# AidaDSP/aidadsp-lv2

Hardware: AMD Instinct MI355X
Metric: audio samples/sec (48 kHz mono, many streams) (higher is better)
Workload: dtype f32; 1 GPU; cfg2: LSTM-32 amp model, 1024 streams/GPU x 256-frame blocks, full run() chain, TTL-default controls; streams_per_gpu=1024, frames=256, kernel=k_lstm_pipe4<32>

## Files before the change

aidadsp-lv2_amd/csrc/aidax_device.h:

```cpp
#pragma once

#include <hip/hip_runtime.h>

#include <cfloat>

#include "aidax_layout.h"

namespace aidax {

__device__ __forceinline__ float dpp_row_shr1(float v)
{
    return __builtin_bit_cast(float, __builtin_amdgcn_update_dpp(0, __builtin_bit_cast(int, v), 0x111, 0xf, 0xf, true));
}

template <int CTRL, int ROW_MASK>
__device__ __forceinline__ float dpp_take(float v)
{
    return __builtin_bit_cast(float, __builtin_amdgcn_update_dpp(0, __builtin_bit_cast(int, v), CTRL, ROW_MASK, 0xf, ROW_MASK == 0xf));
}

__device__ __forceinline__ float wave_sum(float v)
{
    v = v + dpp_take<0xB1, 0xf>(v);
    v = v + dpp_take<0x4E, 0xf>(v);
    v = v + dpp_take<0x141, 0xf>(v);
    v = v + dpp_take<0x140, 0xf>(v);
    v = v + dpp_take<0x142, 0xa>(v);
    v = v + dpp_take<0x143, 0xc>(v);
    return __builtin_bit_cast(float, __builtin_amdgcn_readlane(__builtin_bit_cast(int, v), 63));
}

template <int N>
__device__ __forceinline__ void fmac_row_ror(float& acc, float h, float w)
{
    static_assert(N >= 1 && N <= 15, "rotation within a row of 16 lanes");
    asm volatile("v_fmac_f32_dpp %0, %1, %2 row_ror:%3 row_mask:0xf bank_mask:0xf" : "+v"(acc) : "v"(h), "v"(w), "n"(N));
}

#define AIDAX_ROR1(N, W) "v_fmac_f32_dpp %0, %1, %" #W " row_ror:" #N " row_mask:0xf bank_mask:0xf\n\t"
__device__ __forceinline__ void fmac_row_ror_1_15(float& a0, float h, const float* w)
{
    asm volatile(AIDAX_ROR1(1, 2) AIDAX_ROR1(2, 3) AIDAX_ROR1(3, 4) AIDAX_ROR1(4, 5) AIDAX_ROR1(5, 6) AIDAX_ROR1(6, 7) AIDAX_ROR1(7, 8)
                 AIDAX_ROR1(8, 9) AIDAX_ROR1(9, 10) AIDAX_ROR1(10, 11) AIDAX_ROR1(11, 12) AIDAX_ROR1(12, 13) AIDAX_ROR1(13, 14)
                 AIDAX_ROR1(14, 15) AIDAX_ROR1(15, 16)
                 : "+v"(a0)
                 : "v"(h), "v"(w[1]), "v"(w[2]), "v"(w[3]), "v"(w[4]), "v"(w[5]), "v"(w[6]), "v"(w[7]), "v"(w[8]), "v"(w[9]),
                   "v"(w[10]), "v"(w[11]), "v"(w[12]), "v"(w[13]), "v"(w[14]), "v"(w[15]));
}
#undef AIDAX_ROR1

typedef float aidax_f32x2 __attribute__((ext_vector_type(2)));
#define AIDAX_PKA(ACC, W, HQ) "v_pk_fma_f32 %" #ACC ", %" #W ", %" #HQ ", %" #ACC " op_sel_hi:[1,0,1]\n\t"
#define AIDAX_PKB(ACC, W, HQ) "v_pk_fma_f32 %" #ACC ", %" #W ", %" #HQ ", %" #ACC " op_sel:[0,1,0] op_sel_hi:[1,1,1]\n\t"
#define AIDAX_PKA0(ACC, W, HQ) "v_pk_fma_f32 %" #ACC ", %" #W ", %" #HQ ", 0 op_sel_hi:[1,0,0]\n\t"
#define AIDAX_PKB0(ACC, W, HQ) "v_pk_fma_f32 %" #ACC ", %" #W ", %" #HQ ", 0 op_sel:[0,1,0] op_sel_hi:[1,1,0]\n\t"
__device__ __forceinline__ aidax_f32x2 pk_fma_lds16(aidax_f32x2 pA, const aidax_f32x2* w, const aidax_f32x2* hq)
{
    aidax_f32x2 pB, pC, pD;
    asm volatile(AIDAX_PKA(0, 4, 20) AIDAX_PKB0(1, 5, 20) AIDAX_PKA0(2, 6, 21) AIDAX_PKB0(3, 7, 21)
                 AIDAX_PKA(0, 8, 22) AIDAX_PKB(1, 9, 22) AIDAX_PKA(2, 10, 23) AIDAX_PKB(3, 11, 23)
                 AIDAX_PKA(0, 12, 24) AIDAX_PKB(1, 13, 24) AIDAX_PKA(2, 14, 25) AIDAX_PKB(3, 15, 25)
                 AIDAX_PKA(0, 16, 26) AIDAX_PKB(1, 17, 26) AIDAX_PKA(2, 18, 27) AIDAX_PKB(3, 19, 27)
                 "v_pk_add_f32 %0, %0, %1\n\t"
                 "v_pk_add_f32 %2, %2, %3"
                 : "+v"(pA), "=&v"(pB), "=&v"(pC), "=&v"(pD)
                 : "v"(w[0]), "v"(w[1]), "v"(w[2]), "v"(w[3]), "v"(w[4]), "v"(w[5]), "v"(w[6]), "v"(w[7]), "v"(w[8]), "v"(w[9]), "v"(w[10]),
                   "v"(w[11]), "v"(w[12]), "v"(w[13]), "v"(w[14]), "v"(w[15]),
                   "v"(hq[0]), "v"(hq[1]), "v"(hq[2]), "v"(hq[3]), "v"(hq[4]), "v"(hq[5]), "v"(hq[6]), "v"(hq[7]));
    return pA + pC;
}
#undef AIDAX_PKA
#undef AIDAX_PKB
#undef AIDAX_PKA0
#undef AIDAX_PKB0

struct Pair { float lo, hi; };

__device__ __forceinline__ Pair share_halves(float v)
{
    const unsigned u = __builtin_bit_cast(unsigned, v);
    const auto r = __builtin_amdgcn_permlane32_swap(u, u, false, false);
    const unsigned r0 = r[0], r1 = r[1];
    return { __builtin_bit_cast(float, r0), __builtin_bit_cast(float, r1) };
}

__device__ __forceinline__ Pair share_rows(float v)
{
    const unsigned u = __builtin_bit_cast(unsigned, v);
    const auto r = __builtin_amdgcn_permlane16_swap(u, u, false, false);
    const unsigned r0 = r[0], r1 = r[1];
    return { __builtin_bit_cast(float, r0), __builtin_bit_cast(float, r1) };
}

__device__ __forceinline__ float fast_sigmoid(float v)
{
    const float e = __builtin_amdgcn_exp2f(v * -1.44269504088896340736f);
    return __builtin_amdgcn_rcpf(1.0f + e);
}

constexpr float kNegLog2e = -1.44269504088896340736f;
__device__ __forceinline__ float sigmoid_pre(float v_scaled)
{
    return __builtin_amdgcn_rcpf(1.0f + __builtin_amdgcn_exp2f(v_scaled));
}


constexpr float kTanhP[7] = { 0.9999999933888696f, 0.13084010352004496f, 0.003103956503888039f, 1.1154311501654368e-05f,
                              -2.0225239996482085e-08f, 5.277955823366522e-11f, -8.488730763828322e-14f };
constexpr float kTanhQ[4] = { 1.0f, 0.46417337453820245f, 0.02449517952619233f, 0.00025461456545097517f };
constexpr float kTanhClamp = 0x1.f9b3c2p+2f;
__device__ __forceinline__ float tanh_rat_clamp(float v) { return __builtin_fminf(__builtin_fmaxf(v, -kTanhClamp), kTanhClamp); }
template <bool kUFirst = false>
__device__ __forceinline__ float tanh_rat(float v)
{
    const float x = tanh_rat_clamp(v);
    const float u = x * x;
#ifndef AIDAX_TANH_PLAIN
    typedef float f32x2_t __attribute__((ext_vector_type(2)));
    const f32x2_t uu = { u, u };
    auto step = [&](f32x2_t pq, f32x2_t c) { return kUFirst ? __builtin_elementwise_fma(uu, pq, c) : __builtin_elementwise_fma(pq, uu, c); };
    f32x2_t pq = { kTanhP[6], kTanhQ[3] };
    pq = step(pq, f32x2_t{ kTanhP[5], kTanhQ[2] });
    pq = step(pq, f32x2_t{ kTanhP[4], kTanhQ[1] });
    pq = step(pq, f32x2_t{ kTanhP[3], kTanhQ[0] });
    float pp = pq.x;
    pp = __builtin_fmaf(pp, u, kTanhP[2]);
    pp = __builtin_fmaf(pp, u, kTanhP[1]);
    pp = __builtin_fmaf(pp, u, kTanhP[0]);
    return (pp * x) * __builtin_amdgcn_rcpf(pq.y);
#endif
    float p = kTanhP[6];
    p = __builtin_fmaf(p, u, kTanhP[5]);
    p = __builtin_fmaf(p, u, kTanhP[4]);
    p = __builtin_fmaf(p, u, kTanhP[3]);
    p = __builtin_fmaf(p, u, kTanhP[2]);
    p = __builtin_fmaf(p, u, kTanhP[1]);
    p = __builtin_fmaf(p, u, kTanhP[0]);
    float q = kTanhQ[3];
    q = __builtin_fmaf(q, u, kTanhQ[2]);
    q = __builtin_fmaf(q, u, kTanhQ[1]);
    q = __builtin_fmaf(q, u, kTanhQ[0]);
    return (p * x) * __builtin_amdgcn_rcpf(q);
}

__device__ __forceinline__ float tanh_exp(float v)
{
    const float e = __builtin_amdgcn_exp2f(v * 2.88539008177792681472f);
    return __builtin_fmaf(-2.0f, __builtin_amdgcn_rcpf(1.0f + e), 1.0f);
}

__device__ __forceinline__ float tanh_exp_pre(float v_scaled)
{
    return __builtin_fmaf(-2.0f, __builtin_amdgcn_rcpf(1.0f + __builtin_amdgcn_exp2f(v_scaled)), 1.0f);
}

struct ExpRamp {
    float mem, coef, tc;
    __device__ __forceinline__ void arm(float m, float target, float c)
    {
        mem = m; coef = c; tc = target * (1.f - c);
    }
    __device__ __forceinline__ float next() { mem = mem * coef + tc; return mem; }
};

__device__ __forceinline__ float lin_next(float& mem, float target, float step)
{
    const float y0 = mem;
    const float dy = target - y0;
    mem = y0 + __builtin_copysignf(__builtin_fminf(__builtin_fabsf(dy), __builtin_fabsf(step)), dy);
    return mem;
}

__device__ __forceinline__ bool eq_stage_transparent(double a0, double a1, double a2, double b1, double b2, double z1, double z2)
{
    return a0 == 1.0 && a1 == b1 && a2 == b2 && z1 == 0.0 && z2 == 0.0;
}
__device__ __forceinline__ float eq_skip_sample(float y, float& p)
{
    const float o = y + p;
    p = p + (y - y);
    return o;
}

struct ChainPass {
    int K, gain_lane;
    bool active;
    double a0, a1, a2, b1, b2, z1, z2;
    ExpRamp g;
    bool eq_skip;
    float eq_p;
};

template <int DST_STRIDE, bool CHECK>
__device__ __forceinline__ void chain_step(ChainPass& c, int stage, bool run, bool writer, float head, float& carry,
                                           float* dst, int s, int n)
{
    const float from_left = dpp_row_shr1(carry);
    const float x = stage == 0 ? head : from_left;
// ... 453 lines not shown
```

aidadsp-lv2_amd/csrc/aidax_kernels.hip:

```cpp
#include <hip/hip_runtime.h>
#include <hip/hip_ext.h>

#include <cfloat>

#include <mutex>
#include "aidax_device.h"
#include "aidax_kernels.h"
#include "aidax_layout.h"

namespace aidax {

template <int H, bool ROTP = true>
struct LstmCell {
    static constexpr LaneMap M = lstm_map(H);
    static constexpr int S = M.S, SLOTS = M.slots, NU = M.NU, GPL = M.GPL;
    static constexpr int PACK = lstm_pack_regs(H);
    static constexpr int STATE = 2 * H;
    static constexpr bool ROT4 = ROTP && lstm_rot4(H);
    static constexpr int KW = lstm_row_weights(H, ROT4);

    float w[NU][GPL][KW];
    typedef float f32x2 __attribute__((ext_vector_type(2)));
    f32x2 wl2[16];
    float wx[NU][GPL][kMaxInputs];
    float bias[NU][GPL];
    float wd[NU], bd;
    float aka[GPL], akb[GPL];
    float c[NU], h[NU];
    int part, slot;
#ifdef AIDAX_PIPE_TRACE
    unsigned long long ts6 = 0;
    unsigned long long ts[6];
#define PT_STAMP(k) do { if constexpr (TR) { __builtin_amdgcn_sched_barrier(0); ts[k] = __builtin_amdgcn_s_memtime(); __builtin_amdgcn_sched_barrier(0); } } while (0)
#else
#define PT_STAMP(k) do { } while (0)
#endif
    static constexpr int kStatePart = S == 2 ? 1 : 0;
    static constexpr bool ROT = ROTP && lstm_rot2(H);
    static constexpr int kPackOffset = (!ROTP && lstm_has_alt_pack(H)) ? lstm_alt_pack_offset(H) : 0;

    __device__ __forceinline__ void load(const float* __restrict__ wbase, const float* __restrict__ st, int lane)
    {
        const float* __restrict__ wp = wbase + kPackOffset;
        part = lane / SLOTS;
        slot = lane % SLOTS;
        int r = 0;
#pragma unroll
        for (int m = 0; m < NU; ++m)
#pragma unroll
            for (int e = 0; e < GPL; ++e) {
#pragma unroll
                for (int k = 0; k < KW; ++k) w[m][e][k] = wp[(r++) * kWave + lane];
#pragma unroll
                for (int i = 0; i < kMaxInputs; ++i) wx[m][e][i] = wp[(r++) * kWave + lane];
                bias[m][e] = wp[(r++) * kWave + lane];
            }
#pragma unroll
        for (int m = 0; m < NU; ++m) wd[m] = wp[(r++) * kWave + lane];
        bd = wp[(r++) * kWave + lane];
        if constexpr (ROTP && lstm_rot2(H)) {
            constexpr int kRow = KW + kMaxInputs + 1;
#pragma unroll
            for (int k = 0; k < 16; ++k) wl2[k] = f32x2{ wp[(16 + k) * kWave + lane], wp[(kRow + 16 + k) * kWave + lane] };
        }
#pragma unroll
        for (int e = 0; e < GPL; ++e) {
            const bool is_tanh = (part + S * e) == 2;
            aka[e] = is_tanh ? 1.f : 0.5f;
            akb[e] = is_tanh ? 0.f : 0.5f;
        }
#pragma unroll
        for (int m = 0; m < NU; ++m) {
            const int j = slot + m * SLOTS;
            h[m] = j < H ? st[j] : 0.f;
            c[m] = j < H ? st[H + j] : 0.f;
        }
    }

    __device__ __forceinline__ void store(float* __restrict__ st) const
    {
#pragma unroll
        for (int m = 0; m < NU; ++m) {
            const int j = slot + m * SLOTS;
            if (part == kStatePart && j < H) { st[j] = h[m]; st[H + j] = c[m]; }
        }
    }

    __device__ __forceinline__ void publish_h(float* hbuf) const
    {
#pragma unroll
        for (int m = 0; m < NU; ++m) {
            const int j = slot + m * SLOTS;
            if constexpr (S == 2 && !ROT) {
                if (j < H) hbuf[part == kStatePart ? j : H] = h[m];
            } else {
                if (j < H) hbuf[j] = h[m];
            }
        }
    }

    static constexpr int HID = H;

    __device__ __forceinline__ float dense_partial() const
    {
        float d = 0.f;
#pragma unroll
        for (int m = 0; m < NU; ++m) d = __builtin_fmaf(wd[m], h[m], d);
        return d;
    }

    template <int NI = kMaxInputs, int WINDOW = 0, bool TR = false>
    __device__ __forceinline__ void step(float x0, float x1, float x2, const float* hprev, float* hout)
    {
        PT_STAMP(0);
        float acc[NU][GPL];
#pragma unroll
        for (int m = 0; m < NU; ++m)
#pragma unroll
            for (int e = 0; e < GPL; ++e) {
                float a = bias[m][e];
                a = __builtin_fmaf(wx[m][e][0], x0, a);
                if constexpr (NI >= 2) a = __builtin_fmaf(wx[m][e][1], x1, a);
                if constexpr (NI >= 3) a = __builtin_fmaf(wx[m][e][2], x2, a);
                acc[m][e] = a;
            }
        if constexpr (ROT4) {
            const float hr = h[0];
            float a0 = __builtin_fmaf(w[0][0][0], hr, acc[0][0]);
            fmac_row_ror_1_15(a0, hr, w[0][0]);
            acc[0][0] = a0;
            (void)hprev;
        } else if constexpr (ROT) {
            const float4* hv = reinterpret_cast<const float4*>(hprev + 16 * (1 - ((slot >> 4) & 1)));
            const float4 q0 = hv[0], q1 = hv[1], q2 = hv[2], q3 = hv[3];
            __builtin_amdgcn_sched_barrier(0);
            const float hr = h[0];
            float a0 = acc[0][0], a1 = acc[0][1];
            a0 = __builtin_fmaf(w[0][0][0], hr, a0);
            a1 = __builtin_fmaf(w[0][1][0], hr, a1);
            fmac_row_ror_1_15(a0, hr, w[0][0]);
            fmac_row_ror_1_15(a1, hr, w[0][1]);
            __builtin_amdgcn_s_waitcnt(0xc07f);
            PT_STAMP(1);
            const f32x2 hq[8] = { f32x2{ q0.x, q0.y }, f32x2{ q0.z, q0.w }, f32x2{ q1.x, q1.y }, f32x2{ q1.z, q1.w },
                                  f32x2{ q2.x, q2.y }, f32x2{ q2.z, q2.w }, f32x2{ q3.x, q3.y }, f32x2{ q3.z, q3.w } };
            const f32x2 a01 = pk_fma_lds16(f32x2{ a0, a1 }, wl2, hq);
            acc[0][0] = a01.x; acc[0][1] = a01.y;
            PT_STAMP(2);
        } else {
        const float4* hv = reinterpret_cast<const float4*>(hprev);
#pragma unroll
        for (int k4 = 0; k4 < H / 4; ++k4) {
            const float4 q = hv[k4];
#pragma unroll
            for (int m = 0; m < NU; ++m)
#pragma unroll
                for (int e = 0; e < GPL; ++e) {
                    float a = acc[m][e];
                    a = __builtin_fmaf(w[m][e][4 * k4 + 0], q.x, a);
                    a = __builtin_fmaf(w[m][e][4 * k4 + 1], q.y, a);
                    a = __builtin_fmaf(w[m][e][4 * k4 + 2], q.z, a);
                    a = __builtin_fmaf(w[m][e][4 * k4 + 3], q.w, a);
                    acc[m][e] = a;
                }
            if constexpr (WINDOW > 0) { if ((k4 + 1) % WINDOW == 0) __builtin_amdgcn_sched_barrier(0); }
        }
        }
        __builtin_amdgcn_wave_barrier();
#pragma unroll
        for (int m = 0; m < NU; ++m) {
            float act[GPL];
#pragma unroll
            for (int e = 0; e < GPL; ++e) {
                if constexpr (S == 1) {
                    act[e] = e == 2 ? tanh_rat<ROT>(acc[m][e]) : sigmoid_pre(acc[m][e]);
                } else if (S == 2 && e == 0) {
                    act[e] = sigmoid_pre(acc[m][e]);
                } else {
                    act[e] = __builtin_fmaf(tanh_rat<ROT>(acc[m][e]), aka[e], akb[e]);
                }
            }
            PT_STAMP(3);
            float gi_gg, gf, go;
            if constexpr (S == 1) {
                gi_gg = act[0] * act[2]; gf = act[1]; go = act[3];
            } else if constexpr (S == 2) {
                const float ig = act[0] * act[1];
                const auto r = __builtin_amdgcn_permlane32_swap(__builtin_bit_cast(unsigned, acc[m][1]), __builtin_bit_cast(unsigned, ig), false, false);
                const unsigned r0 = r[0];
                gi_gg = __builtin_bit_cast(float, r0); gf = act[0]; go = act[1];
            } else {
                const Pair p = share_halves(act[0]);
                const Pair lo = share_rows(p.lo), hi = share_rows(p.hi);
                gi_gg = lo.lo * hi.lo; gf = lo.hi; go = hi.hi;
            }
            const float cn = __builtin_fmaf(gf, c[m], gi_gg);
            c[m] = cn;
#ifdef AIDAX_TANHC_EXP
            const float hn = go * tanh_exp(cn);
#else
            const float hn = go * tanh_rat<ROT>(cn);
#endif
            if constexpr (ROT) h[m] = share_halves(hn).hi;
            else h[m] = hn;
        }
        PT_STAMP(4);
        publish_h(hout);
        __builtin_amdgcn_wave_barrier();
        PT_STAMP(5);
    }
};

template <int H>
struct GruCell {
    static constexpr LaneMap M = gru_map(H);
    static constexpr int S = M.S, SLOTS = M.slots, NU = M.NU;
    static constexpr int KS = H / S;
    static constexpr int PACK = gru_pack_regs(H);
    static constexpr int STATE = H;
#ifdef AIDAX_PIPE_TRACE
    unsigned long long ts6 = 0, ts[6] = { 0, 0, 0, 0, 0, 0 };
#endif
    static_assert(KS % 4 == 0, "K slice must stay float4 aligned");

    float w[NU][3][KS];
    float wx[NU][3][kMaxInputs];
    float bias[NU][3];
    float bn1[NU];
    float wd[NU], bd;
    float h[NU];
    int part, slot;

    __device__ __forceinline__ void load(const float* __restrict__ wp, const float* __restrict__ st, int lane)
    {
        part = lane / SLOTS;
        slot = lane % SLOTS;
        int r = 0;
#pragma unroll
        for (int m = 0; m < NU; ++m)
#pragma unroll
            for (int e = 0; e < 3; ++e) {
#pragma unroll
                for (int k = 0; k < KS; ++k) w[m][e][k] = wp[(r++) * kWave + lane];
#pragma unroll
                for (int i = 0; i < kMaxInputs; ++i) wx[m][e][i] = wp[(r++) * kWave + lane];
                bias[m][e] = wp[(r++) * kWave + lane];
            }
#pragma unroll
        for (int m = 0; m < NU; ++m) bn1[m] = wp[(r++) * kWave + lane];
#pragma unroll
        for (int m = 0; m < NU; ++m) wd[m] = wp[(r++) * kWave + lane];
        bd = wp[(r++) * kWave + lane];
#pragma unroll
        for (int m = 0; m < NU; ++m) {
            const int j = slot + m * SLOTS;
            h[m] = j < H ? st[j] : 0.f;
        }
    }

    __device__ __forceinline__ void store(float* __restrict__ st) const
    {
#pragma unroll
        for (int m = 0; m < NU; ++m) {
            const int j = slot + m * SLOTS;
            if (part == 0 && j < H) st[j] = h[m];
        }
    }

    __device__ __forceinline__ void publish_h(float* hbuf) const
    {
#pragma unroll
        for (int m = 0; m < NU; ++m) {
            const int j = slot + m * SLOTS;
            if (j < H) hbuf[j] = h[m];
        }
    }

    static constexpr int HID = H;

    __device__ __forceinline__ float dense_partial() const
    {
        float d = 0.f;
#pragma unroll
        for (int m = 0; m < NU; ++m) d = __builtin_fmaf(wd[m], h[m], d);
        return d;
    }

    __device__ __forceinline__ static float unit_sum(float v)
    {
        if constexpr (S == 1) return v;
        else if constexpr (S == 2) { const Pair p = share_halves(v); return p.lo + p.hi; }
        else { const Pair p = share_halves(v); const float t = p.lo + p.hi; const Pair q = share_rows(t); return q.lo + q.hi; }
    }

    template <int NI = kMaxInputs, int WINDOW = 0, bool TR = false>
    __device__ __forceinline__ void step(float x0, float x1, float x2, const float* hprev, float* hout)
    {
        float ax[NU][3], ar[NU][3];
#pragma unroll
        for (int m = 0; m < NU; ++m)
#pragma unroll
            for (int e = 0; e < 3; ++e) {
// ... 630 lines not shown
    float* hh = rows + kP4Streams * n;
    float* hand = hh + kP4Streams * kRing * HS;
    float* wdl = hand + kP4HandFloats;
    int* prog = reinterpret_cast<int*>(wdl + H + 4);
    float* hstate = reinterpret_cast<float*>(prog + 8);
    float* prow = hstate + 5 * kWave;
    const int I = kCond ? (int)a.input_size : 1;

    int Kp = 1;
#ifdef AIDAX_P4_BARRIER
    int Kq = 1;
#endif
    uint32_t fw[kP4Streams];
#pragma unroll
    for (int j = 0; j < kP4Streams; ++j) {
        const int jc = s0 + j < (int)a.n_streams ? s0 + j : (int)a.n_streams - 1;
        const uint32_t f = a.ctl[jc].flags;
        fw[j] = s0 + j < (int)a.n_streams ? f : 0u;
        if ((f & CTL_EQ_PRE) && s0 + j < (int)a.n_streams) Kp = 6;
#ifdef AIDAX_P4_BARRIER
        if ((f & CTL_EQ_POST) && s0 + j < (int)a.n_streams) Kq = 6;
#endif
    }
    const int d1 = Kp / 2 + 1;
#ifdef AIDAX_P4_BARRIER
    const int T = (n / B - 1 + (Kq - 1) + 2 * (d1 + 1)) / 2 + 1;
#endif

    if (wave < kP4Streams) {
        const int s = s0 + wave;
        const int sc = s < (int)a.n_streams ? s : (int)a.n_streams - 1;
        float* nnst = a.nn + (size_t)sc * a.nn_stride;
        float* hj = hh + wave * kRing * HS;
        const float* row = rows + wave * n;
        Cell cell;
        if (!(AIDAX_TUNE(a) & 1)) __builtin_amdgcn_s_setprio(3);
        cell.load(a.wpack, nnst, lane);
        P4_STAMP(1);
        const uint32_t fl = wave == 0 ? fw[0] : wave == 1 ? fw[1] : wave == 2 ? fw[2] : fw[3];
        const bool net = (fl & (CTL_ENABLED | CTL_NET_ON)) == (CTL_ENABLED | CTL_NET_ON);
        cell.publish_h(hj + (kRing - 1) * HS);
        __syncthreads();
        P4_STAMP(2);
#ifndef AIDAX_P4_BARRIER
        if (!net) { p4_post(prog + 2 + wave, NT, lane); return; }
#endif
#ifdef AIDAX_P4_BARRIER
        for (int tick = 0; tick < T; ++tick) {
            const int t = tick - d1;
            for (int i = 0; i < wave * ((AIDAX_TUNE(a) >> 24) & 3); ++i) asm volatile("s_nop 15");
            if (t >= 0 && t < NT) {
#else
        for (int i = 0; i < wave * ((AIDAX_TUNE(a) >> 24) & 15); ++i) asm volatile("s_nop 15");
        p4_i2 ahead = p4_i2{ 0, 0 };
        for (int t = 0; t < NT; ++t) {
            if (ahead.x <= t || ahead.y < t - 1)
                while (p4_peek(prog) <= t || p4_peek(prog + 1) < t - 1) __builtin_amdgcn_s_sleep(1);
#ifdef AIDAX_P4_TRACE
            if (t == 0) P4_STAMP(3);
            if (t == 1) P4_STAMP(4);
            if (t == NT - 1) P4_STAMP(5);
            if (wave == 0 && t < 32) {
                __builtin_amdgcn_sched_barrier(0);
                const unsigned long long now = __builtin_amdgcn_s_memrealtime();
                if (lane == 0) reinterpret_cast<unsigned long long*>(hstate)[8 + t] = now;
                __builtin_amdgcn_sched_barrier(0);
            }
#endif
            {
#endif
                const int base = t * kSB;
                const float* hprev = hj + ((base + kRing - 1) & (kRing - 1)) * HS;
                float* hcur = hj + (base & (kRing - 1)) * HS;
                const float* xs = row + base;
                float xr[kSB];
                asm volatile(".p2align 6");
                auto fetch_x = [&](int q) {
                    const float4 v = reinterpret_cast<const float4*>(xs)[q];
                    xr[4 * q] = v.x; xr[4 * q + 1] = v.y;
                    xr[4 * q + 2] = v.z; xr[4 * q + 3] = v.w;
                };
                fetch_x(0);
                if constexpr (!kCond) {
#pragma unroll
                    for (int f = 0; f < kSB; ++f) {
                        if ((f & 3) == 1 && f / 4 + 1 < kSB / 4) fetch_x(f / 4 + 1);
#ifndef AIDAX_P4_BARRIER
                        if (f == kSB - 4) ahead = *(const volatile p4_lds_i2*)(const p4_lds_i2*)(prog);
#endif
                        cell.template step<1>(xr[f], 0.f, 0.f, f == 0 ? hprev : hcur + (f - 1) * HS, hcur + f * HS);
                    }
                } else {
                    const float* p1s = prow + (wave * 2 + 0) * n + base;
                    const float* p2s = prow + (wave * 2 + 1) * n + base;
                    float p1r[kSB], p2r[kSB];
                    auto fetch_p = [&](int q) {
                        const float4 u = reinterpret_cast<const float4*>(p1s)[q];
                        const float4 w = reinterpret_cast<const float4*>(p2s)[q];
                        p1r[4 * q] = u.x; p1r[4 * q + 1] = u.y; p1r[4 * q + 2] = u.z; p1r[4 * q + 3] = u.w;
                        p2r[4 * q] = w.x; p2r[4 * q + 1] = w.y; p2r[4 * q + 2] = w.z; p2r[4 * q + 3] = w.w;
                    };
                    fetch_p(0);
#pragma unroll
                    for (int f = 0; f < kSB; ++f) {
                        if ((f & 3) == 1 && f / 4 + 1 < kSB / 4) { fetch_x(f / 4 + 1); fetch_p(f / 4 + 1); }
#ifndef AIDAX_P4_BARRIER
                        if (f == kSB - 4) ahead = *(const volatile p4_lds_i2*)(const p4_lds_i2*)(prog);
#endif
                        cell.template step<3>(xr[f], p1r[f], I >= 3 ? p2r[f] : 0.f, f == 0 ? hprev : hcur + (f - 1) * HS, hcur + f * HS);
                    }
                }
            }
#ifdef AIDAX_P4_BARRIER
            __syncthreads();
#else
            p4_post(prog + 2 + wave, t + 1, lane);
#endif
        }
        P4_STAMP(6);
        cell.store(nnst);
#ifdef AIDAX_P4_TRACE
        P4_STAMP(7);
        {
            unsigned long long mine = 0;
#pragma unroll
            for (int k = 0; k < 8; ++k) if (lane == k) mine = tr[k];
            if (wave == 0 && lane < 8) reinterpret_cast<unsigned long long*>(hstate)[lane] = mine;
        }
#endif
        return;
    }

    const int hq = wave - kP4Streams;
    const int j = lane < kP4ChainLanes ? lane / 12 : kP4Streams - 1;
    const int r = lane - 12 * (lane / 12);
    const bool isQ = r >= 6;
    const int stage = isQ ? r - 6 : r;
    const bool there = s0 + j < (int)a.n_streams;
    const int sj = there ? s0 + j : (int)a.n_streams - 1;
    const StreamCtl& ctl = a.ctl[sj];
    StreamState& st = a.st[sj];
    const int slot = isQ ? post_slot(stage) : pre_slot(stage);
    float4 r0 = float4{0.f, 0.f, 0.f, 0.f}, r1 = r0, r2 = r0, r3 = r0;
    if (kP4Helpers == 1 && n == 256) {
        const bool t1 = s0 + 1 < (int)a.n_streams, t2 = s0 + 2 < (int)a.n_streams, t3 = s0 + 3 < (int)a.n_streams;
        r0 = reinterpret_cast<const float4*>(a.in + (size_t)s0 * n)[lane];
        r1 = reinterpret_cast<const float4*>(a.in + (size_t)(t1 ? s0 + 1 : s0) * n)[lane];
        r2 = reinterpret_cast<const float4*>(a.in + (size_t)(t2 ? s0 + 2 : s0) * n)[lane];
        r3 = reinterpret_cast<const float4*>(a.in + (size_t)(t3 ? s0 + 3 : s0) * n)[lane];
    } else if (kP4Helpers == 1 && n < 256) {
        const int have4 = ((int)a.n_streams - s0 < kP4Streams ? (int)a.n_streams - s0 : kP4Streams) * (n / 4);
        const float4* g4 = reinterpret_cast<const float4*>(a.in + (size_t)s0 * n);
        const int i0 = lane, i1 = kWave + lane, i2 = 2 * kWave + lane, i3 = 3 * kWave + lane;
        r0 = g4[i0 < have4 ? i0 : 0];
        r1 = g4[i1 < have4 ? i1 : 0];
        r2 = g4[i2 < have4 ? i2 : 0];
        r3 = g4[i3 < have4 ? i3 : 0];
    }
    static_assert(H + 1 <= kWave, "the Dense's weights and bias: a lane each");
    const float* wd_nat = a.wpack + (size_t)Cell::PACK * kWave;
    const float wdv = wd_nat[lane < H + 1 ? lane : 0];
    ChainPass c;
    chain_load(c, ctl, st, slot, false);
    const uint32_t flags = ctl.flags;
    uint32_t pending = st.pending;
    float pre_mem = st.pre_mem, master_mem = st.master_mem, pre_tgt = st.pre_tgt, master_tgt = st.master_tgt;
    const float ctl_pre_target = ctl.pre_target, ctl_master_target = ctl.master_target, ctl_pre_coef = ctl.pre_coef, ctl_master_coef = ctl.master_coef;
    const int dj = lane >> 4, df = lane & 15;
    const uint32_t fdj = a.ctl[s0 + dj < (int)a.n_streams ? s0 + dj : (int)a.n_streams - 1].flags;
    static_assert(kP4Helpers == 1, "the PARAM lanes' state is not handed from helper to helper");
    const bool plane = kCond && lane >= kP4ChainLanes && lane < kP4ChainLanes + 2 * kP4Streams;
    const int jp = plane ? (lane - kP4ChainLanes) >> 1 : 0, ip = lane & 1;
// ... 138 lines not shown
            if (netd) drow[f] = drow[f] * a.in_gain;
            __builtin_amdgcn_wave_barrier();
            p4_post(prog, ts + 1, lane);
        }
#ifdef AIDAX_P4_BARRIER
        __syncthreads();
#endif
        if (kP4Helpers > 1 && tick + 1 < T) {
            double* zs = reinterpret_cast<double*>(hstate);
            zs[lane] = c.z1; zs[kWave + lane] = c.z2;
            hstate[4 * kWave + lane] = g.mem;
            __builtin_amdgcn_wave_barrier();
            p4_post(prog + 6, tick + 1, lane);
        }
    }
    P4_STAMP(5);
    if ((T - 1) % kP4Helpers != hq) return;
    if (is_gain) c.g = g;
    if (!run || !c.active) { c.z1 = z1o; c.z2 = z2o; }
    if (run) { st.z[slot][0] = c.z1; st.z[slot][1] = c.z2; }
    {
        const float pj = __builtin_bit_cast(float, __builtin_amdgcn_ds_bpermute(4 * (lane - stage), __builtin_bit_cast(int, c.eq_p)));
        if (skipj && live && lane < kP4ChainLanes && isQ && stage >= 1 && pj != pj) {
            st.z[slot][0] = __builtin_nan("");
            st.z[slot][1] = __builtin_nan("");
        }
    }
#ifdef AIDAX_TEST_HOOKS
    if (there && lane < kP4ChainLanes && r == 6) st.pad = (uint32_t)Kqj;
#endif
    if (there && lane < kP4ChainLanes && !isQ && stage == 0) { st.pre_mem = c.g.mem; st.pre_tgt = pre_tgt; }
    if (there && lane < kP4ChainLanes && isQ && stage == c.K - 1) { st.master_mem = c.g.mem; st.master_tgt = master_tgt; }
    if constexpr (kCond) {
        if (there && lane < kP4ChainLanes && r == 0) st.pending = netj ? (pending & ~PEND_PARAM_FIRST) : pending;
        if (net_p) { a.st[sp].p_mem[ip] = pm; a.st[sp].p_tgt[ip] = pt; a.st[sp].p_step[ip] = ps; }
    } else {
        if (there && lane < kP4ChainLanes && r == 0) st.pending = netj ? param_targets(ctl, st, pending) : pending;
    }
    if (n == 256) {
        const float4 r0 = reinterpret_cast<const float4*>(rows)[lane], r1 = reinterpret_cast<const float4*>(rows + n)[lane];
        const float4 r2 = reinterpret_cast<const float4*>(rows + 2 * n)[lane], r3 = reinterpret_cast<const float4*>(rows + 3 * n)[lane];
        reinterpret_cast<float4*>(a.out + (size_t)s0 * n)[lane] = r0;
        if (s0 + 1 < (int)a.n_streams) reinterpret_cast<float4*>(a.out + (size_t)(s0 + 1) * n)[lane] = r1;
        if (s0 + 2 < (int)a.n_streams) reinterpret_cast<float4*>(a.out + (size_t)(s0 + 2) * n)[lane] = r2;
        if (s0 + 3 < (int)a.n_streams) reinterpret_cast<float4*>(a.out + (size_t)(s0 + 3) * n)[lane] = r3;
    } else if (kP4Helpers == 1 && n < 256) {
        const int have4 = ((int)a.n_streams - s0 < kP4Streams ? (int)a.n_streams - s0 : kP4Streams) * (n / 4);
        const float4* l4 = reinterpret_cast<const float4*>(rows);
        float4* o4 = reinterpret_cast<float4*>(a.out + (size_t)s0 * n);
#pragma unroll
        for (int k = 0; k < 4; ++k) {
            const int i = k * kWave + lane;
            if (i < have4) o4[i] = l4[i];
        }
    } else {
        for (int jj = 0; jj < kP4Streams; ++jj) {
            if (s0 + jj >= (int)a.n_streams) break;
            float4* dst = reinterpret_cast<float4*>(a.out + (size_t)(s0 + jj) * n);
            const float4* src = reinterpret_cast<const float4*>(rows + jj * n);
            for (int i = lane; i < n / 4; i += kWave) dst[i] = src[i];
        }
    }
    post_done_word(a, lane);
#ifdef AIDAX_P4_TRACE
    P4_STAMP(6);
    asm volatile("s_waitcnt vmcnt(0)" ::: "memory");
    P4_STAMP(7);
    if (n >= 64) {
        unsigned long long* dst = reinterpret_cast<unsigned long long*>(a.out + (size_t)s0 * n);
        if (lane < 8) dst[lane] = reinterpret_cast<const unsigned long long*>(hstate)[lane];
        unsigned long long mine = 0;
#pragma unroll
        for (int k = 0; k < 8; ++k) if (lane == k) mine = tr[k];
        if (lane < 8) dst[8 + lane] = mine;
        if (lane < 32 && lane < NT && 16 + lane < n / 2) dst[16 + lane] = reinterpret_cast<const unsigned long long*>(hstate)[8 + lane];
    }
#endif
}

template <int H, bool kCond = false>
__global__ __launch_bounds__(kP4Waves * kWave) void k_lstm_pipe4(LaunchArgs a)
{
    extern __shared__ __attribute__((aligned(16))) float smem[];
    stream_body_pipe4<LstmCell<H>, kCond>(a, smem);
}

template <int H, bool kCond = false>
__global__ __launch_bounds__(kP4Waves * kWave) void k_gru_pipe4(LaunchArgs a)
{
    extern __shared__ __attribute__((aligned(16))) float smem[];
    stream_body_pipe4<GruCell<H>, kCond>(a, smem);
}

constexpr int kChainStreams = 8;

template <bool PRE>
__global__ __launch_bounds__(kWave) void k_chain(LaunchArgs a)
{
    extern __shared__ __attribute__((aligned(16))) float smem[];
    const int lane = threadIdx.x;
    const int n = (int)a.n_frames;
    const int nP = (n + 3) & ~3;
    for (int g = 0; g < kChainStreams; ++g) {
        const int s2 = blockIdx.x * kChainStreams + g;
        if (s2 < (int)a.n_streams && n != 0)
            load_block(smem + g * nP, (PRE ? a.in : a.out) + (size_t)s2 * n, n, lane);
    }
    __builtin_amdgcn_wave_barrier();
    chain_wave_pass<PRE>(a, blockIdx.x * kChainStreams, smem, nP, smem + kChainStreams * nP, n, lane, true, false);
    if (n != 0) {
        for (int g = 0; g < kChainStreams; ++g) {
            const int s2 = blockIdx.x * kChainStreams + g;
            if (s2 >= (int)a.n_streams) continue;
            const bool row_live = (a.ctl[s2].flags & CTL_ENABLED) != 0;
            if (PRE ? (row_live || a.out != a.in) : row_live)
                store_block(a.out + (size_t)s2 * n, smem + g * nP, n, lane);
        }
    }
}

constexpr int kNnSub = 16;
constexpr int kNnRing = 2 * kNnSub;
constexpr int kNnWindow = 4;

__host__ __device__ constexpr size_t nn_lds_floats(int H, int n_frames)
{
    return (size_t)((n_frames + 3) & ~3) + (size_t)kNnRing * pipe_row_stride(H) + (size_t)(H + 4);
}

template <class Cell>
__global__ __launch_bounds__(kWave) void k_nn(LaunchArgs a)
{
    extern __shared__ __attribute__((aligned(16))) float smem[];
    constexpr int H = Cell::HID;
    constexpr int HS = pipe_row_stride(H);
    const int lane = threadIdx.x;
    const int s = blockIdx.x;
    const int n = (int)a.n_frames;
    const StreamCtl& ctl = a.ctl[s];
    StreamState& st = a.st[s];
    const uint32_t flags = ctl.flags;
    if (n == 0 || !(flags & CTL_ENABLED) || !(flags & CTL_NET_ON)) return;

    float* buf = smem;
    float* hh = smem + ((n + 3) & ~3);
    float* wdl = hh + kNnRing * HS;
    float* row = a.out + (size_t)s * n;
    load_block(buf, row, n, lane);
    const float* wd_nat = a.wpack + (size_t)Cell::PACK * kWave;
    for (int i = lane; i < H + 1; i += kWave) wdl[i] = wd_nat[i];

    float p_mem[2] = { st.p_mem[0], st.p_mem[1] };
    float p_tgt[2] = { st.p_tgt[0], st.p_tgt[1] };
    float p_step[2] = { st.p_step[0], st.p_step[1] };
    uint32_t pending = st.pending;
#pragma unroll
    for (int i = 0; i < 2; ++i) {
        const float nt = ctl.p_target[i];
        if (__builtin_fabsf(p_tgt[i] - nt) >= FLT_EPSILON) {
            p_tgt[i] = nt;
            p_step[i] = (p_tgt[i] - p_mem[i]) / ctl.p_den;
        }
    }
    if (pending & PEND_PARAM_FIRST) {
        pending &= ~PEND_PARAM_FIRST;
        p_mem[0] = p_tgt[0];
        p_mem[1] = p_tgt[1];
// ... 368 lines not shown
```

Measured before the change: 4.673 billion samples/s.

## Pair LSTM-32 gate preactivations with packed FMA and precompute next-frame input term

For the H=32 unconditioned LSTM pipeline kernel, the per-gate bias and input-weight terms are packed into f32x2 registers and the input contribution for the next frame is computed early, overlapped after the LDS packed-FMA chain. The first recurrent FMA becomes a packed FMA, the output multiply is fused with the permlane32 swap in inline asm, and tanh clamping uses fmed3. The aim is to shorten the serial per-frame critical path of the recurrence. In exchange it adds register pressure from the held partial sums and hand-scheduled asm with sched barriers that could disturb the existing schedule.

```diff
diff --git a/aidadsp-lv2_amd/csrc/aidax_device.h b/aidadsp-lv2_amd/csrc/aidax_device.h
--- a/aidadsp-lv2_amd/csrc/aidax_device.h
+++ b/aidadsp-lv2_amd/csrc/aidax_device.h
@@ -54,21 +54,30 @@
 #define AIDAX_PKB(ACC, W, HQ) "v_pk_fma_f32 %" #ACC ", %" #W ", %" #HQ ", %" #ACC " op_sel:[0,1,0] op_sel_hi:[1,1,1]\n\t"
 #define AIDAX_PKA0(ACC, W, HQ) "v_pk_fma_f32 %" #ACC ", %" #W ", %" #HQ ", 0 op_sel_hi:[1,0,0]\n\t"
 #define AIDAX_PKB0(ACC, W, HQ) "v_pk_fma_f32 %" #ACC ", %" #W ", %" #HQ ", 0 op_sel:[0,1,0] op_sel_hi:[1,1,0]\n\t"
+#define AIDAX_PK16_LINKS AIDAX_PKA(0, 4, 20) AIDAX_PKB0(1, 5, 20) AIDAX_PKA0(2, 6, 21) AIDAX_PKB0(3, 7, 21)                                         \
+                         AIDAX_PKA(0, 8, 22) AIDAX_PKB(1, 9, 22) AIDAX_PKA(2, 10, 23) AIDAX_PKB(3, 11, 23)                                            \
+                         AIDAX_PKA(0, 12, 24) AIDAX_PKB(1, 13, 24) AIDAX_PKA(2, 14, 25) AIDAX_PKB(3, 15, 25)                                          \
+                         AIDAX_PKA(0, 16, 26) AIDAX_PKB(1, 17, 26) AIDAX_PKA(2, 18, 27) AIDAX_PKB(3, 19, 27)                                          \
+                         "v_pk_add_f32 %0, %0, %1\n\t"                                                                                                \
+                         "v_pk_add_f32 %2, %2, %3"
+#define AIDAX_PK16_OPERANDS : "+v"(pA), "=&v"(pB), "=&v"(pC), "=&v"(pD)                                                                                  \
+                 : "v"(w[0]), "v"(w[1]), "v"(w[2]), "v"(w[3]), "v"(w[4]), "v"(w[5]), "v"(w[6]), "v"(w[7]), "v"(w[8]), "v"(w[9]), "v"(w[10]),          \
+                   "v"(w[11]), "v"(w[12]), "v"(w[13]), "v"(w[14]), "v"(w[15]),                                                                         \
+                   "v"(hq[0]), "v"(hq[1]), "v"(hq[2]), "v"(hq[3]), "v"(hq[4]), "v"(hq[5]), "v"(hq[6]), "v"(hq[7])
 __device__ __forceinline__ aidax_f32x2 pk_fma_lds16(aidax_f32x2 pA, const aidax_f32x2* w, const aidax_f32x2* hq)
 {
     aidax_f32x2 pB, pC, pD;
-    asm volatile(AIDAX_PKA(0, 4, 20) AIDAX_PKB0(1, 5, 20) AIDAX_PKA0(2, 6, 21) AIDAX_PKB0(3, 7, 21)
-                 AIDAX_PKA(0, 8, 22) AIDAX_PKB(1, 9, 22) AIDAX_PKA(2, 10, 23) AIDAX_PKB(3, 11, 23)
-                 AIDAX_PKA(0, 12, 24) AIDAX_PKB(1, 13, 24) AIDAX_PKA(2, 14, 25) AIDAX_PKB(3, 15, 25)
-                 AIDAX_PKA(0, 16, 26) AIDAX_PKB(1, 17, 26) AIDAX_PKA(2, 18, 27) AIDAX_PKB(3, 19, 27)
-                 "v_pk_add_f32 %0, %0, %1\n\t"
-                 "v_pk_add_f32 %2, %2, %3"
-                 : "+v"(pA), "=&v"(pB), "=&v"(pC), "=&v"(pD)
-                 : "v"(w[0]), "v"(w[1]), "v"(w[2]), "v"(w[3]), "v"(w[4]), "v"(w[5]), "v"(w[6]), "v"(w[7]), "v"(w[8]), "v"(w[9]), "v"(w[10]),
-                   "v"(w[11]), "v"(w[12]), "v"(w[13]), "v"(w[14]), "v"(w[15]),
-                   "v"(hq[0]), "v"(hq[1]), "v"(hq[2]), "v"(hq[3]), "v"(hq[4]), "v"(hq[5]), "v"(hq[6]), "v"(hq[7]));
+    asm volatile(AIDAX_PK16_LINKS AIDAX_PK16_OPERANDS);
     return pA + pC;
 }
+__device__ __forceinline__ aidax_f32x2 pk_fma_lds16_sum(aidax_f32x2 pA, const aidax_f32x2* w, const aidax_f32x2* hq, aidax_f32x2& pB, aidax_f32x2& pC, aidax_f32x2& pD)
+{
+    asm volatile(AIDAX_PK16_LINKS "\n\tv_pk_add_f32 %0, %0, %2" AIDAX_PK16_OPERANDS);
+    return pA;
+}
+__device__ __forceinline__ void pk_hold(aidax_f32x2 pB, aidax_f32x2 pC, aidax_f32x2 pD) { asm volatile("" : : "v"(pB), "v"(pC), "v"(pD)); }
+#undef AIDAX_PK16_LINKS
+#undef AIDAX_PK16_OPERANDS
 #undef AIDAX_PKA
 #undef AIDAX_PKB
 #undef AIDAX_PKA0
@@ -82,6 +91,21 @@
     const auto r = __builtin_amdgcn_permlane32_swap(u, u, false, false);
     const unsigned r0 = r[0], r1 = r[1];
     return { __builtin_bit_cast(float, r0), __builtin_bit_cast(float, r1) };
+}
+
+__device__ __forceinline__ float mul_share_halves_hi(float go, float t)
+{
+    typedef float f32x2_t __attribute__((ext_vector_type(2)));
+    f32x2_t gp, tp;
+    gp.x = go; tp.x = t;
+    float lo, hi;
+    asm volatile("v_pk_mul_f32 v[2:3], %2, %3 op_sel_hi:[0,0]\n\t"
+                 "s_nop 1\n\t"
+                 "v_permlane32_swap_b32 v3, v2"
+                 : "={v3}"(lo), "={v2}"(hi)
+                 : "v"(gp), "v"(tp));
+    (void)lo;
+    return hi;
 }
 
 __device__ __forceinline__ Pair share_rows(float v)
@@ -110,10 +134,10 @@
 constexpr float kTanhQ[4] = { 1.0f, 0.46417337453820245f, 0.02449517952619233f, 0.00025461456545097517f };
 constexpr float kTanhClamp = 0x1.f9b3c2p+2f;
 __device__ __forceinline__ float tanh_rat_clamp(float v) { return __builtin_fminf(__builtin_fmaxf(v, -kTanhClamp), kTanhClamp); }
-template <bool kUFirst = false>
+template <bool kUFirst = false, bool kMed3 = false>
 __device__ __forceinline__ float tanh_rat(float v)
 {
-    const float x = tanh_rat_clamp(v);
+    const float x = kMed3 ? __builtin_amdgcn_fmed3f(v, -kTanhClamp, kTanhClamp) : tanh_rat_clamp(v);
     const float u = x * x;
 #ifndef AIDAX_TANH_PLAIN
     typedef float f32x2_t __attribute__((ext_vector_type(2)));
diff --git a/aidadsp-lv2_amd/csrc/aidax_kernels.hip b/aidadsp-lv2_amd/csrc/aidax_kernels.hip
--- a/aidadsp-lv2_amd/csrc/aidax_kernels.hip
+++ b/aidadsp-lv2_amd/csrc/aidax_kernels.hip
@@ -10,18 +10,20 @@
 
 namespace aidax {
 
-template <int H, bool ROTP = true>
+template <int H, bool ROTP = true, bool PAIRS = false>
 struct LstmCell {
     static constexpr LaneMap M = lstm_map(H);
     static constexpr int S = M.S, SLOTS = M.slots, NU = M.NU, GPL = M.GPL;
     static constexpr int PACK = lstm_pack_regs(H);
     static constexpr int STATE = 2 * H;
+    static constexpr bool kPairs = PAIRS;
     static constexpr bool ROT4 = ROTP && lstm_rot4(H);
     static constexpr int KW = lstm_row_weights(H, ROT4);
 
     float w[NU][GPL][KW];
     typedef float f32x2 __attribute__((ext_vector_type(2)));
     f32x2 wl2[16];
+    f32x2 w02, wx2, b2, ain;
     float wx[NU][GPL][kMaxInputs];
     float bias[NU][GPL];
     float wd[NU], bd;
@@ -62,6 +64,11 @@
             constexpr int kRow = KW + kMaxInputs + 1;
 #pragma unroll
             for (int k = 0; k < 16; ++k) wl2[k] = f32x2{ wp[(16 + k) * kWave + lane], wp[(kRow + 16 + k) * kWave + lane] };
+            if constexpr (PAIRS) {
+                w02 = f32x2{ wp[lane], wp[kRow * kWave + lane] };
+                wx2 = f32x2{ wp[KW * kWave + lane], wp[(kRow + KW) * kWave + lane] };
+                b2 = f32x2{ wp[(KW + kMaxInputs) * kWave + lane], wp[(kRow + KW + kMaxInputs) * kWave + lane] };
+            }
         }
 #pragma unroll
         for (int e = 0; e < GPL; ++e) {
@@ -109,15 +116,20 @@
         return d;
     }
 
-    template <int NI = kMaxInputs, int WINDOW = 0, bool TR = false>
-    __device__ __forceinline__ void step(float x0, float x1, float x2, const float* hprev, float* hout)
+    template <int hi>
+    __device__ __forceinline__ void input_pair(f32x2 xp) { ain = __builtin_elementwise_fma(__builtin_shufflevector(xp, xp, hi, hi), wx2, b2); }
+
+    template <int NI = kMaxInputs, int WINDOW = 0, bool TR = false, bool NEXT = false, int kNextHi = 0>
+    __device__ __forceinline__ void step(float x0, float x1, float x2, const float* hprev, float* hout, f32x2 xn = f32x2{ 0.f, 0.f })
     {
         PT_STAMP(0);
         float acc[NU][GPL];
+        static_assert(!PAIRS || (ROTP && lstm_rot2(H) && NI == 1), "the paired frame is the ROT frame of a one-input model");
 #pragma unroll
         for (int m = 0; m < NU; ++m)
 #pragma unroll
             for (int e = 0; e < GPL; ++e) {
+                if constexpr (PAIRS) { acc[m][e] = 0.f; continue; }
                 float a = bias[m][e];
                 a = __builtin_fmaf(wx[m][e][0], x0, a);
                 if constexpr (NI >= 2) a = __builtin_fmaf(wx[m][e][1], x1, a);
@@ -136,16 +148,29 @@
             __builtin_amdgcn_sched_barrier(0);
             const float hr = h[0];
             float a0 = acc[0][0], a1 = acc[0][1];
+            if constexpr (PAIRS) {
+                const f32x2 a = __builtin_elementwise_fma(f32x2{ hr, hr }, w02, ain);
+                a0 = a.x; a1 = a.y;
+            } else {
             a0 = __builtin_fmaf(w[0][0][0], hr, a0);
             a1 = __builtin_fmaf(w[0][1][0], hr, a1);
+            }
             fmac_row_ror_1_15(a0, hr, w[0][0]);
             fmac_row_ror_1_15(a1, hr, w[0][1]);
             __builtin_amdgcn_s_waitcnt(0xc07f);
             PT_STAMP(1);
             const f32x2 hq[8] = { f32x2{ q0.x, q0.y }, f32x2{ q0.z, q0.w }, f32x2{ q1.x, q1.y }, f32x2{ q1.z, q1.w },
                                   f32x2{ q2.x, q2.y }, f32x2{ q2.z, q2.w }, f32x2{ q3.x, q3.y }, f32x2{ q3.z, q3.w } };
-            const f32x2 a01 = pk_fma_lds16(f32x2{ a0, a1 }, wl2, hq);
+            f32x2 a01, pB, pC, pD;
+            if constexpr (PAIRS) a01 = pk_fma_lds16_sum(f32x2{ a0, a1 }, wl2, hq, pB, pC, pD);
+            else a01 = pk_fma_lds16(f32x2{ a0, a1 }, wl2, hq);
             acc[0][0] = a01.x; acc[0][1] = a01.y;
+            if constexpr (PAIRS && NEXT) {
+                __builtin_amdgcn_sched_barrier(0);
+                input_pair<kNextHi>(xn);
+                pk_hold(pB, pC, pD);
+                __builtin_amdgcn_sched_barrier(0);
+            }
             PT_STAMP(2);
         } else {
         const float4* hv = reinterpret_cast<const float4*>(hprev);
@@ -177,7 +202,7 @@
                 } else if (S == 2 && e == 0) {
                     act[e] = sigmoid_pre(acc[m][e]);
                 } else {
-                    act[e] = __builtin_fmaf(tanh_rat<ROT>(acc[m][e]), aka[e], akb[e]);
+                    act[e] = __builtin_fmaf(tanh_rat<ROT, PAIRS>(acc[m][e]), aka[e], akb[e]);
                 }
             }
             PT_STAMP(3);
@@ -197,12 +222,17 @@
             const float cn = __builtin_fmaf(gf, c[m], gi_gg);
             c[m] = cn;
 #ifdef AIDAX_TANHC_EXP
-            const float hn = go * tanh_exp(cn);
+            const float th = tanh_exp(cn);
 #else
-            const float hn = go * tanh_rat<ROT>(cn);
-#endif
-            if constexpr (ROT) h[m] = share_halves(hn).hi;
-            else h[m] = hn;
+            const float th = tanh_rat<ROT>(cn);
+#endif
+            if constexpr (PAIRS) {
+                h[m] = mul_share_halves_hi(go, th);
+            } else {
+                const float hn = go * th;
+                if constexpr (ROT) h[m] = share_halves(hn).hi;
+                else h[m] = hn;
+            }
         }
         PT_STAMP(4);
         publish_h(hout);
@@ -218,6 +248,7 @@
     static constexpr int KS = H / S;
     static constexpr int PACK = gru_pack_regs(H);
     static constexpr int STATE = H;
+    static constexpr bool kPairs = false;
 #ifdef AIDAX_PIPE_TRACE
     unsigned long long ts6 = 0, ts[6] = { 0, 0, 0, 0, 0, 0 };
 #endif
@@ -1014,12 +1045,19 @@
                 };
                 fetch_x(0);
                 if constexpr (!kCond) {
+                    typedef float f32x2 __attribute__((ext_vector_type(2)));
+                    if constexpr (Cell::kPairs) cell.template input_pair<0>(f32x2{ xr[0], xr[1] });
 #pragma unroll
                     for (int f = 0; f < kSB; ++f) {
                         if ((f & 3) == 1 && f / 4 + 1 < kSB / 4) fetch_x(f / 4 + 1);
 #ifndef AIDAX_P4_BARRIER
                         if (f == kSB - 4) ahead = *(const volatile p4_lds_i2*)(const p4_lds_i2*)(prog);
 #endif
+                        if constexpr (Cell::kPairs) {
+                            if (f + 1 < kSB && (f & 1)) cell.template step<1, 0, false, true, 0>(xr[f], 0.f, 0.f, f == 0 ? hprev : hcur + (f - 1) * HS, hcur + f * HS, f32x2{ xr[f + 1], xr[(f + 2) % kSB] });
+                            else if (f + 1 < kSB) cell.template step<1, 0, false, true, 1>(xr[f], 0.f, 0.f, f == 0 ? hprev : hcur + (f - 1) * HS, hcur + f * HS, f32x2{ xr[f], xr[f + 1] });
+                            else cell.template step<1>(xr[f], 0.f, 0.f, f == 0 ? hprev : hcur + (f - 1) * HS, hcur + f * HS);
+                        } else
                         cell.template step<1>(xr[f], 0.f, 0.f, f == 0 ? hprev : hcur + (f - 1) * HS, hcur + f * HS);
                     }
                 } else {
@@ -1324,7 +1362,7 @@
 __global__ __launch_bounds__(kP4Waves * kWave) void k_lstm_pipe4(LaunchArgs a)
 {
     extern __shared__ __attribute__((aligned(16))) float smem[];
-    stream_body_pipe4<LstmCell<H>, kCond>(a, smem);
+    stream_body_pipe4<LstmCell<H, true, H == 32 && !kCond>, kCond>(a, smem);
 }
 
 template <int H, bool kCond = false>
```

After: 4.738 billion samples/s, median of 6. +1.4%, better.
